# ViskaWei/VIT

Measured on AMD Instinct MI355X. Metric: images/sec ViT-B/16 224^2 bf16 train step, higher is better.
Workload: dtype bf16

## Files before the change

### vit_amd/csrc/gemm2.hip

```cpp
#include <algorithm>
#include <stdio.h>

#include "common.h"

namespace vit {

#define GLB_AS __attribute__((address_space(1)))

struct Gemm2Args {
  const char* A; const char* B; char* C;
  long lda, ldb, ldc;
  int M, N, K;
  int tiles_m, tiles_n, nblk;
  int splits, k_per_split;
  float* slab;
  const float* bias;
  const short* aux_in; short* aux_out; long ldaux;
  const float* residual; long ldres;
  float alpha;
  int act, c_dtype;
  DropCfg drop;
  int rpb, orb, roff;
  int drs;
  int lin_split;
  float* colsum_part;
  int grp2;
  const float* rope_cos; const float* rope_sin;
  int rope_T, rope_dh, rope_cols;
};

__device__ __forceinline__ int tr_swz2(int k) { return ((k & 3) | (((k >> 3) & 1) << 2)) << 2; }

template <int WM, int WN, int CW, int EPI>
__device__ __forceinline__ void tile_epilogue(f32x4 (&acc)[WM][WN], char* scr, const Gemm2Args& p, int m0, int n0,
                                              int split, int lane) {
  const int l15 = lane & 15, lg = lane >> 4;
  constexpr int CPR = CW / 4;
  constexpr int RPI = 64 / CPR;
  float* slab = p.splits > 1 ? p.slab + (long)split * p.M * p.N : nullptr;
#pragma unroll
  for (int i = 0; i < WM; ++i) {
#pragma unroll
    for (int jc = 0; jc < (WN * 16) / CW; ++jc) {
#pragma unroll
      for (int jj = 0; jj < CW / 16; ++jj) {
        const int c16 = jj * 4 + lg;
        *(f32x4*)(scr + l15 * (CW * 4) + ((c16 ^ (l15 & (CPR - 1))) << 4)) = acc[i][jc * (CW / 16) + jj];
        acc[i][jc * (CW / 16) + jj] = (f32x4){0.f, 0.f, 0.f, 0.f};
      }
#pragma unroll
      for (int rr = 0; rr < 16 / RPI; ++rr) {
        const int row = rr * RPI + lane / CPR, c16 = lane % CPR;
        f32x4 v = *(const f32x4*)(scr + row * (CW * 4) + ((c16 ^ (row & (CPR - 1))) << 4));
        const int m = m0 + i * 16 + row, n = n0 + jc * CW + c16 * 4;
        if (slab) {
          *(f32x4*)(slab + (long)m * p.N + n) = v;
          continue;
        }
        long orow = m;
        if (p.rpb > 0) {
          const int b = m / p.rpb;
          orow = (long)b * p.orb + (m - b * p.rpb) + p.roff;
        }
        v *= p.alpha;
        if (p.bias) v += *(const f32x4*)(p.bias + n);
        if (EPI == 1) {
          f32x4 sv = v;
          if (p.act == VIT_ACT_GELU_GRAD) {
#pragma unroll
            for (int r = 0; r < 4; ++r) {
              float g_, d_;
              gelu_both(v[r], g_, d_);
              v[r] = g_;
              sv[r] = d_;
            }
          } else {
#pragma unroll
            for (int r = 0; r < 4; ++r) v[r] = gelu_erf(v[r]);
          }
          if (p.aux_out) {
            u32x2 pk = {pack2bf(sv[0], sv[1]), pack2bf(sv[2], sv[3])};
            *(u32x2*)(p.aux_out + orow * p.ldaux + n) = pk;
          }
        } else if (EPI == 2) {
          bf16x4 u = *(const bf16x4*)(p.aux_in + orow * p.ldaux + n);
          if (p.act == VIT_ACT_MUL_AUX) {
#pragma unroll
            for (int r = 0; r < 4; ++r) v[r] *= bf2f(u[r]);
          } else {
#pragma unroll
            for (int r = 0; r < 4; ++r) v[r] *= dgelu_erf(bf2f(u[r]));
          }
        }
        if (p.drop.thr) {
          float k0, k1, k2, k3;
          const unsigned long long krow = (unsigned long long)orow * (unsigned)p.drs;
          drop_pair(p.drop, krow, (unsigned)n, k0, k1);
          drop_pair(p.drop, krow, (unsigned)n + 2, k2, k3);
          v[0] *= k0; v[1] *= k1; v[2] *= k2; v[3] *= k3;
        }
        if (p.residual) v += *(const f32x4*)(p.residual + orow * p.ldres + n);
        if (p.c_dtype == VIT_BF16) {
          u32x2 pk = {pack2bf(v[0], v[1]), pack2bf(v[2], v[3])};
          *(u32x2*)(p.C + (orow * p.ldc + n) * 2) = pk;
        } else {
          *(f32x4*)(p.C + (orow * p.ldc + n) * 4) = v;
        }
      }
    }
  }
}

int launch_splitk_reduce(const float* slab, float* C, long ldc, int M, int N, int splits, float alpha, int accumulate,
                         hipStream_t st);

template <int FAST, int NI>
__device__ __forceinline__ void pp_epilogue(f32x4 (&acc)[NI][4], char* scr, const Gemm2Args& p, int m0, int n0, int split,
                                            int lane) {
  const int l15 = lane & 15, lg = lane >> 4;
  if (FAST == 7) {
    float* cf = p.splits > 1 ? p.slab + (long)split * p.M * p.N : (float*)p.C;
    const long ldc = p.splits > 1 ? (long)p.N : p.ldc;
    const int n = n0 + l15 * 4;
#pragma unroll
    for (int i = 0; i < NI; ++i) {
#pragma unroll
      for (int j = 0; j < 4; ++j) {
        *(f32x4*)(scr + l15 * 256 + (((j * 4 + lg) ^ l15) << 4)) = acc[i][j];
        acc[i][j] = (f32x4){0.f, 0.f, 0.f, 0.f};
      }
#pragma unroll
      for (int rr = 0; rr < 4; ++rr) {
        const int row = rr * 4 + lg;
        *(f32x4*)(cf + (long)(m0 + i * 16 + row) * ldc + n) = *(const f32x4*)(scr + row * 256 + ((l15 ^ row) << 4));
      }
    }
    return;
  }
  const int cg = lane & 7, rsub = lane >> 3;
  const int n = n0 + cg * 8;
  const __amdgpu_buffer_rsrc_t rc_ = make_rsrc(p.C, (unsigned long long)p.M * p.ldc * 2);
  const __amdgpu_buffer_rsrc_t ra_ = make_rsrc(p.aux_out ? (const void*)p.aux_out : (const void*)p.C, (unsigned long long)p.M * p.ldaux * 2);
#define EPI_STORE_C(M_, PK) __builtin_amdgcn_raw_buffer_store_b128(PK, rc_, (unsigned)(((M_) * p.ldc + n) * 2), 0, 16)
#define EPI_STORE_AUX(M_, PK) __builtin_amdgcn_raw_buffer_store_b128(PK, ra_, (unsigned)(((M_) * p.ldaux + n) * 2), 0, 16)
  f32x4 bv0 = (f32x4){0.f, 0.f, 0.f, 0.f}, bv1 = bv0;
  if ((FAST == 3 || FAST == 4 || FAST == 8) && p.bias) {
    bv0 = *(const f32x4*)(p.bias + n);
    bv1 = *(const f32x4*)(p.bias + n + 4);
  }
  float cs[8] = {0.f, 0.f, 0.f, 0.f, 0.f, 0.f, 0.f, 0.f};
  const bool want_cs = p.colsum_part != nullptr;
  u32x4 au[4][2];
  f32x4 rc0, rc1, rs0, rs1, k8c0, k8c1, k8s0, k8s1;
  int rt = 0;
  const int rope_peer = (lane ^ (p.rope_dh >> 4)) << 2;
  if (FAST == 8 && n0 < p.rope_cols) {
    const int hl_ = p.rope_dh >> 4, hd = p.rope_dh >> 1, io = (cg & (hl_ - 1)) * 8;
    rt = (m0 + rsub) % p.rope_T;
    const long to = (long)rt * hd + io, t8 = 8L * hd + io;
    rc0 = *(const f32x4*)(p.rope_cos + to); rc1 = *(const f32x4*)(p.rope_cos + to + 4);
    rs0 = *(const f32x4*)(p.rope_sin + to); rs1 = *(const f32x4*)(p.rope_sin + to + 4);
    k8c0 = *(const f32x4*)(p.rope_cos + t8); k8c1 = *(const f32x4*)(p.rope_cos + t8 + 4);
    k8s0 = *(const f32x4*)(p.rope_sin + t8); k8s1 = *(const f32x4*)(p.rope_sin + t8 + 4);
  }
  const __amdgpu_buffer_rsrc_t rx_ = make_rsrc(p.aux_in ? (const void*)p.aux_in : (const void*)p.C, (unsigned long long)p.M * p.ldaux * 2);
#pragma unroll
  for (int i = 0; i < NI; ++i) {
    if (FAST == 5 && (i & 3) == 0) {
#pragma unroll
      for (int ii = 0; ii < 4; ++ii)
#pragma unroll
        for (int rr = 0; rr < 2; ++rr)
          au[ii][rr] = __builtin_amdgcn_raw_buffer_load_b128(rx_, (unsigned)(((long)(m0 + (i + ii) * 16 + rr * 8 + rsub) * p.ldaux + n) * 2), 0, 18);
    }
    f32x4 v[2][2];
#pragma unroll
    for (int j = 0; j < 4; ++j) {
      *(f32x4*)(scr + l15 * 256 + (((j * 4 + lg) ^ l15) << 4)) = acc[i][j];
      acc[i][j] = (f32x4){0.f, 0.f, 0.f, 0.f};
    }
#pragma unroll
    for (int rr = 0; rr < 2; ++rr) {
      const int row = rr * 8 + rsub;
      v[rr][0] = *(const f32x4*)(scr + row * 256 + (((2 * cg) ^ row) << 4));
      v[rr][1] = *(const f32x4*)(scr + row * 256 + (((2 * cg + 1) ^ row) << 4));
    }
#pragma unroll
    for (int rr = 0; rr < 2; ++rr) {
      const long m = m0 + i * 16 + rr * 8 + rsub;
      float o[8];
#pragma unroll
      for (int r = 0; r < 4; ++r) {
        o[r] = v[rr][0][r] + bv0[r];
        o[4 + r] = v[rr][1][r] + bv1[r];
      }
      if (FAST == 4) {
        float sv[8];
        if (p.act == VIT_ACT_GELU_GRAD) {
#pragma unroll
          for (int r = 0; r < 8; r += 2) {
            f32x2 g_, d_;
            gelu_both2((f32x2){o[r], o[r + 1]}, g_, d_);
            o[r] = g_[0]; o[r + 1] = g_[1];
            sv[r] = d_[0]; sv[r + 1] = d_[1];
          }
        } else {
#pragma unroll
          for (int r = 0; r < 8; r += 2) {
            sv[r] = o[r]; sv[r + 1] = o[r + 1];
            const f32x2 g_ = gelu_erf2((f32x2){o[r], o[r + 1]});
            o[r] = g_[0]; o[r + 1] = g_[1];
          }
        }
        if (p.aux_out) {
          u32x4 pk = {pack2bf(sv[0], sv[1]), pack2bf(sv[2], sv[3]), pack2bf(sv[4], sv[5]), pack2bf(sv[6], sv[7])};
          EPI_STORE_AUX(m, pk);
        }
      }
      if (FAST == 5) {
        const u32x4 u = au[i & 3][rr];
        if (p.act == VIT_ACT_MUL_AUX) {
#pragma unroll
          for (int r = 0; r < 4; ++r) {
            o[2 * r] *= __builtin_bit_cast(float, u[r] << 16);
            o[2 * r + 1] *= __builtin_bit_cast(float, u[r] & 0xFFFF0000u);
          }
        } else {
#pragma unroll
          for (int r = 0; r < 4; ++r) {
            o[2 * r] *= dgelu_erf(__builtin_bit_cast(float, u[r] << 16));
            o[2 * r + 1] *= dgelu_erf(__builtin_bit_cast(float, u[r] & 0xFFFF0000u));
          }
        }
      }
      if (FAST == 8 && n0 < p.rope_cols) {
        const int hl = p.rope_dh >> 4;
        const float sg = (cg & hl) ? 1.f : -1.f;
        const f32x4 c0 = rc0, c1 = rc1, s0 = rs0, s1 = rs1;
        float px[8];
#pragma unroll
        for (int r = 0; r < 8; ++r)
          px[r] = __builtin_bit_cast(float, __builtin_amdgcn_ds_bpermute(rope_peer, __builtin_bit_cast(int, o[r])));
#pragma unroll
        for (int r = 0; r < 4; ++r) {
          o[r] = fmaf(o[r], c0[r], sg * px[r] * s0[r]);
          o[4 + r] = fmaf(o[4 + r], c1[r], sg * px[4 + r] * s1[r]);
        }
        rt += 8;
        const bool wrapped = rt >= p.rope_T;
        if (wrapped) rt -= p.rope_T;
        {
          const f32x4 nc0 = rc0 * k8c0 - rs0 * k8s0, ns0 = rs0 * k8c0 + rc0 * k8s0;
          const f32x4 nc1 = rc1 * k8c1 - rs1 * k8s1, ns1 = rs1 * k8c1 + rc1 * k8s1;
          rc0 = nc0; rs0 = ns0; rc1 = nc1; rs1 = ns1;
        }
        if (__builtin_amdgcn_ballot_w64(wrapped)) {
          const long to = (long)rt * (p.rope_dh >> 1) + (cg & (hl - 1)) * 8;
          rc0 = *(const f32x4*)(p.rope_cos + to); rc1 = *(const f32x4*)(p.rope_cos + to + 4);
          rs0 = *(const f32x4*)(p.rope_sin + to); rs1 = *(const f32x4*)(p.rope_sin + to + 4);
        }
      }
      if (FAST == 3 && p.drop.thr) {
#pragma unroll
        for (int r = 0; r < 4; ++r) {
          float k0, k1;
          drop_pair(p.drop, (unsigned long long)m, (unsigned)n + 2 * r, k0, k1);
          o[2 * r] *= k0;
          o[2 * r + 1] *= k1;
        }
      }
      u32x4 pk = {pack2bf(o[0], o[1]), pack2bf(o[2], o[3]), pack2bf(o[4], o[5]), pack2bf(o[6], o[7])};
      EPI_STORE_C(m, pk);
      if (want_cs) {
#pragma unroll
        for (int r = 0; r < 4; ++r) {
          cs[2 * r] += __builtin_bit_cast(float, pk[r] << 16);
          cs[2 * r + 1] += __builtin_bit_cast(float, pk[r] & 0xFFFF0000u);
        }
      }
    }
  }
  if (p.colsum_part) {
#pragma unroll
    for (int r = 0; r < 8; ++r) {
      float v = cs[r];
      v += __shfl_xor(v, 8, 64);
      v += __shfl_xor(v, 16, 64);
      v += __shfl_xor(v, 32, 64);
      cs[r] = v;
    }
    if (lane < 8) {
      float* dst = p.colsum_part + (long)(m0 >> 7) * p.N + n;
      *(f32x4*)dst = (f32x4){cs[0], cs[1], cs[2], cs[3]};
      *(f32x4*)(dst + 4) = (f32x4){cs[4], cs[5], cs[6], cs[7]};
    }
  }
#undef EPI_STORE_C
#undef EPI_STORE_AUX
}

template <int A_T, int B_T, int EPI, int NSLOT>
__global__ __launch_bounds__(512, 2) void gemm3_kernel(Gemm2Args p) {
  resolve_drop(p.drop);
  constexpr int BM = 256, BN = 256, BK = 64;
  constexpr int HALF = 128 * BK * 2;
  static_assert(NSLOT == 8, "the ring arithmetic below is for 8 slots (two K-tiles of four half-tiles)");
  constexpr int DEPTH = NSLOT - 3, INFL = 2 * (DEPTH - 1);
  constexpr int SCR = 4096, CW = 64;
  constexpr int XA0 = 0, XB0 = 1, XB1 = 2, XA1 = 3;
  constexpr int RELAX = INFL + (((EPI >= 3 && EPI <= 6) || EPI == 8) ? 16 : 32);
  extern __shared__ __attribute__((aligned(16))) char smem[];

  const int tid = threadIdx.x, lane = tid & 63;
  const int wave = __builtin_amdgcn_readfirstlane(tid >> 6);
  const int wr = wave >> 2, wc = wave & 3, grp = wr;
  const int l15 = lane & 15, lg = lane >> 4;

  const int ntile = p.tiles_m * p.tiles_n;
  int split = blockIdx.y, bx = blockIdx.x;
  if (p.lin_split) {
    const int total = ntile * p.splits, lin = blockIdx.x;
    const int q = total >> 3, r = total & 7, xcd = lin & 7, within = lin >> 3;
    const int pos = (xcd < r ? xcd * (q + 1) : r * (q + 1) + (xcd - r) * q) + within;
    split = pos / ntile;
    bx = pos - split * ntile;
  }
  const int k_begin = split * p.k_per_split;
  const int k_end = min(p.K, k_begin + p.k_per_split);
  const int nk = (k_end - k_begin) / BK;
  const int nblk = p.nblk;
  const int my_tiles = (ntile - bx + nblk - 1) / nblk;
  const int T = my_tiles * nk;

  int offA[2], offB[2];
#pragma unroll
  for (int i = 0; i < 2; ++i) {
    if (A_T == 0) {
      const int rimg = i * 64 + wave * 8 + (lane >> 3);
      offA[i] = (i * 128 + wave * 8 + (lane >> 3)) * (int)p.lda + (((lane & 7) ^ ((rimg >> 1) & 7)) << 3);
    } else {
      const int k = i * 32 + wave * 4 + (lane >> 4);
      const int c16 = (lane & 15) ^ (tr_swz2(k) >> 1);
      offA[i] = k * (int)p.lda + (c16 >> 3) * 128 + ((c16 & 7) << 3);
    }
    if (B_T == 0) {
      const int rimg = i * 64 + wave * 8 + (lane >> 3);
      offB[i] = ((rimg >> 5) * 64 + (rimg & 31)) * (int)p.ldb + (((lane & 7) ^ ((rimg >> 1) & 7)) << 3);
    } else {
      const int k = i * 32 + wave * 4 + (lane >> 4);
      const int c16 = (lane & 15) ^ (tr_swz2(k) >> 1);
      offB[i] = k * (int)p.ldb + (c16 >> 2) * 64 + ((c16 & 3) << 3);
    }
  }
  const long halfA = (A_T == 0) ? 64 * p.lda : 64, halfB = (B_T == 0) ? 32 * p.ldb : 32;

  auto tile_coords = [&](int j, int& tm, int& tn) {
    const int round0 = j * nblk;
    const int n_here = min(nblk, ntile - round0);
    const int q = n_here >> 3, r = n_here & 7, xcd = bx & 7, within = bx >> 3;
    const int pos = (xcd < r ? xcd * (q + 1) : r * (q + 1) + (xcd - r) * q) + within;
    if (p.grp2) {
      const int hgrp = n_here >> 1, hn = p.tiles_n >> 1;
      const int g = pos >= hgrp;
      const int u = (round0 >> 1) + (g ? pos - hgrp : pos);
      tm = u / hn;
      tn = g * hn + (u - tm * hn);
      return;
    }
    const int t = p.lin_split ? bx : round0 + pos;
    tm = t / p.tiles_n;
    tn = t - tm * p.tiles_n;
  };
  const long dA = (A_T == 0) ? (long)BK * 2 : (long)BK * p.lda * 2;
  const long dB = (B_T == 0) ? (long)BK * 2 : (long)BK * p.ldb * 2;
  int cj = 0, ckt = 0;
  const char *ca, *cb;
  auto tile_bases = [&](int j) {
    int tm, tn;
    tile_coords(j, tm, tn);
    ca = (A_T == 0) ? p.A + ((long)tm * BM * p.lda + k_begin) * 2 : p.A + ((long)k_begin * p.lda + (long)tm * BM) * 2;
    cb = (B_T == 0) ? p.B + ((long)tn * BN * p.ldb + k_begin) * 2 : p.B + ((long)k_begin * p.ldb + (long)tn * BN) * 2;
  };
  tile_bases(0);
  auto cursor_next = [&](const char*& ab, const char*& bb) {
    ab = ca;
    bb = cb;
    if (++ckt == nk) {
      if (cj + 1 < my_tiles) {
        ++cj;
        ckt = 0;
        tile_bases(cj);
      } else {
        ckt = nk - 1;
      }
    } else {
      ca += dA;
      cb += dB;
    }
  };
  unsigned dofs = 0;
  const unsigned smem_a = lds_addr_of(smem) + wave * 1024;
  auto issue_half = [&](const char* base, long half_off, const int (&off)[2]) {
    const unsigned dst = smem_a + dofs;
    dofs = (dofs + HALF) & (NSLOT * HALF - 1);
    const char* sb = base + half_off * 2;
    lds_dma16_s(sb, (unsigned)off[0] * 2u, dst);
    lds_dma16_s(sb, (unsigned)off[1] * 2u, dst + 8192);
  };

  const int tq = l15 >> 2, tp = l15 & 3;
  const int tr_f = (tq | ((lg & 1) << 2)) << 2;
  int kc_off[2];
#pragma unroll
  for (int s = 0; s < 2; ++s) kc_off[s] = l15 * 128 + (((s * 4 + lg) ^ (l15 >> 1)) << 4);
  auto read_frag = [&](const char* img, int trans, int base16, int s) -> bf16x8 {
    if (!trans) {
      return *(const bf16x8*)(img + base16 * (BK * 2) + kc_off[s]);
    } else {
      const char* pa = img + (s * 32 + lg * 8 + tq) * 256 + ((((base16 >> 2) + tp) ^ tr_f) << 3);
      bf16x4 lo = __builtin_amdgcn_ds_read_tr16_b64_v4i16((LDS_AS bf16x4*)pa);
      bf16x4 hi = __builtin_amdgcn_ds_read_tr16_b64_v4i16((LDS_AS bf16x4*)(pa + 4 * 256));
      return (bf16x8){lo[0], lo[1], lo[2], lo[3], hi[0], hi[1], hi[2], hi[3]};
    }
  };

  f32x4 acc[8][4];
#pragma unroll
  for (int i = 0; i < 8; ++i)
#pragma unroll
    for (int j = 0; j < 4; ++j) acc[i][j] = (f32x4){0.f, 0.f, 0.f, 0.f};
  bf16x8 af[4][2], b0[2][2], b1[2][2];

#define PP_READ_A(IMG)                                                                           \
  _Pragma("unroll") for (int i_ = 0; i_ < 4; ++i_) _Pragma("unroll") for (int s_ = 0; s_ < 2; ++s_) \
      af[i_][s_] = read_frag(IMG, A_T, wr * 64 + i_ * 16, s_);
#define PP_READ_B(BF, IMG)                                                                       \
  _Pragma("unroll") for (int j_ = 0; j_ < 2; ++j_) _Pragma("unroll") for (int s_ = 0; s_ < 2; ++s_) \
      BF[j_][s_] = read_frag(IMG, B_T, wc * 32 + j_ * 16, s_);
#define PP_MFMA(HA, HB, BF)                                                                      \
  __builtin_amdgcn_sched_barrier(0);                                                             \
  __builtin_amdgcn_s_barrier();                                                                  \
  asm volatile("s_waitcnt lgkmcnt(0)" ::: "memory");                                             \
  __builtin_amdgcn_sched_barrier(0);                                                             \
  __builtin_amdgcn_s_setprio(1);                                                                 \
  _Pragma("unroll") for (int s_ = 0; s_ < 2; ++s_) _Pragma("unroll") for (int i_ = 0; i_ < 4; ++i_) \
      _Pragma("unroll") for (int j_ = 0; j_ < 2; ++j_)                                            \
          acc[HA * 4 + i_][HB * 2 + j_] =                                                        \
              __builtin_amdgcn_mfma_f32_16x16x32_bf16(BF[j_][s_], af[i_][s_], acc[HA * 4 + i_][HB * 2 + j_], 0, 0, 0); \
  __builtin_amdgcn_s_setprio(0);                                                                 \
  __builtin_amdgcn_sched_barrier(0);                                                             \
  __builtin_amdgcn_s_barrier();
#define PP_STAGE(BASE, HOFF, OFF)                                                                \
  {                                                                                              \
  issue_half(BASE, HOFF, OFF);                                                                   \
  asm volatile("s_cmp_lg_u32 %0, 0\n\t"                                                          \
               "s_cbranch_scc1 .Lpp_relaxed_%=\n\t"                                              \
               "s_waitcnt vmcnt(%1)\n\t"                                                         \
               "s_branch .Lpp_waited_%=\n"                                                       \
               ".Lpp_relaxed_%=:\n\t"                                                            \
               "s_waitcnt vmcnt(%2)\n"                                                           \
               ".Lpp_waited_%=:" ::"s"(relaxed), "n"(INFL), "n"(RELAX) : "scc", "memory");        \
  }
#define PP_KTILE4                                                                                \
  PP_READ_B(b0, sp + XB0 * HALF)                                                                 \
  PP_READ_A(sp + XA0 * HALF)                                                                     \
  PP_STAGE(bb1, halfB, offB)                                                                     \
  PP_MFMA(0, 0, b0)                                                                              \
  PP_READ_B(b1, sp + XB1 * HALF)                                                                 \
  PP_STAGE(a1, halfA, offA)                                                                      \
  PP_MFMA(0, 1, b1)                                                                              \
  PP_READ_A(sp + XA1 * HALF)                                                                     \
  PP_STAGE(a2, 0, offA)                                                                          \
  PP_MFMA(1, 1, b1)                                                                              \
  PP_STAGE(bb2, 0, offB)                                                                         \
  PP_MFMA(1, 0, b0)
#define PP_LOADED(RX)                                                                            \
  asm volatile("s_cmp_lg_u32 %0, 0\n\t"                                                          \
               "s_cbranch_scc1 .Lpp_relaxed_%=\n\t"                                              \
               "s_waitcnt vmcnt(%1)\n\t"                                                         \
               "s_branch .Lpp_waited_%=\n"                                                       \
               ".Lpp_relaxed_%=:\n\t"                                                            \
               "s_waitcnt vmcnt(%2)\n"                                                           \
               ".Lpp_waited_%=:\n\t"                                                             \
               "s_waitcnt lgkmcnt(0)" ::"s"(relaxed), "n"(INFL), "n"(RX) : "scc", "memory");
#define PP_MFMA2(HA, BFA, HBA, BFB, HBB)                                                         \
  __builtin_amdgcn_sched_barrier(0);                                                             \
  __builtin_amdgcn_s_barrier();                                                                  \
  __builtin_amdgcn_sched_barrier(0);                                                             \
  __builtin_amdgcn_s_setprio(1);                                                                 \
  _Pragma("unroll") for (int s_ = 0; s_ < 2; ++s_) _Pragma("unroll") for (int i_ = 0; i_ < 4; ++i_) \
      _Pragma("unroll") for (int j_ = 0; j_ < 2; ++j_)                                            \
          acc[HA * 4 + i_][HBA * 2 + j_] =                                                       \
              __builtin_amdgcn_mfma_f32_16x16x32_bf16(BFA[j_][s_], af[i_][s_], acc[HA * 4 + i_][HBA * 2 + j_], 0, 0, 0); \
  _Pragma("unroll") for (int s_ = 0; s_ < 2; ++s_) _Pragma("unroll") for (int i_ = 0; i_ < 4; ++i_) \
      _Pragma("unroll") for (int j_ = 0; j_ < 2; ++j_)                                            \
          acc[HA * 4 + i_][HBB * 2 + j_] =                                                       \
              __builtin_amdgcn_mfma_f32_16x16x32_bf16(BFB[j_][s_], af[i_][s_], acc[HA * 4 + i_][HBB * 2 + j_], 0, 0, 0); \
  __builtin_amdgcn_s_setprio(0);                                                                 \
  __builtin_amdgcn_sched_barrier(0);                                                             \
  __builtin_amdgcn_s_barrier();
#define PP_KTILE2                                                                                \
  PP_READ_B(b0, sp + XB0 * HALF)                                                                 \
  PP_READ_A(sp + XA0 * HALF)                                                                     \
  PP_READ_B(b1, sp + XB1 * HALF)                                                                 \
  issue_half(a1, halfA, offA);                                                                   \
  PP_LOADED(RELAX)                                                                               \
  PP_MFMA2(0, b0, 0, b1, 1)                                                                      \
  PP_READ_A(sp + XA1 * HALF)                                                                     \
  issue_half(a2, 0, offA);                                                                       \
  issue_half(bb2, 0, offB);                                                                      \
  issue_half(bb2, halfB, offB);                                                                  \
  PP_LOADED(RELAX)                                                                               \
  PP_MFMA2(1, b1, 1, b0, 0)
  constexpr bool MERGED = A_T || B_T;

  static_assert(DEPTH == 5, "stage schedule written out for the 8-slot ring");
  const char *a1, *bb1, *a2, *bb2;
  {
    const char *a0, *bb0;
    cursor_next(a0, bb0);
    issue_half(a0, 0, offA);
    issue_half(bb0, 0, offB);
    issue_half(bb0, halfB, offB);
    issue_half(a0, halfA, offA);
    cursor_next(a1, bb1);
    issue_half(a1, 0, offA);
    issue_half(bb1, 0, offB);
    if constexpr (MERGED) issue_half(bb1, halfB, offB);
    asm volatile("s_waitcnt vmcnt(%0)" ::"n"(INFL) : "memory");
    cursor_next(a2, bb2);
  }
  __builtin_amdgcn_s_barrier();
  if (grp == 1) __builtin_amdgcn_s_barrier();

  unsigned kb = 0;
  int relaxed = 0;
  for (int jt = 0; jt < my_tiles; ++jt) {
    for (int kt = 0; kt < nk; ++kt) {
      const char* sp = smem + kb;
      if constexpr (MERGED) {
        PP_KTILE2
      } else {
        PP_KTILE4
      }
      relaxed = 0;
      a1 = a2;
      bb1 = bb2;
      cursor_next(a2, bb2);
      kb ^= 4 * HALF;
    }
    {
      int tm, tn;
      tile_coords(jt, tm, tn);
      if (grp == 0) __builtin_amdgcn_s_barrier();
      char* scr = smem + 8 * HALF + wave * SCR;
      if constexpr (EPI >= 3) pp_epilogue<EPI, 8>(acc, scr, p, tm * BM + wr * 128, tn * BN + wc * 64, split, lane);
      else tile_epilogue<8, 4, CW, EPI>(acc, scr, p, tm * BM + wr * 128, tn * BN + wc * 64, split, lane);
      if (grp == 1) __builtin_amdgcn_s_barrier();
      relaxed = 1;
    }
  }
  if (grp == 0) __builtin_amdgcn_s_barrier();
#undef PP_READ_A
#undef PP_READ_B
#undef PP_MFMA
#undef PP_STAGE
#undef PP_KTILE2
#undef PP_KTILE4
#undef PP_LOADED
#undef PP_MFMA2
  asm volatile("s_waitcnt vmcnt(0)" ::: "memory");
}

template <int AT, int BT, int EPI>
static int launch_stag(const Gemm2Args& a, dim3 grid, hipStream_t st) {
  constexpr int smem = 160 * 1024;
  static bool attr_done = false;
  auto fn = gemm3_kernel<AT, BT, EPI, 8>;
  if (!attr_done) {
    VIT_HIP(hipFuncSetAttribute((const void*)fn, hipFuncAttributeMaxDynamicSharedMemorySize, smem));
    attr_done = true;
  }
  hipLaunchKernelGGL(fn, grid, dim3(512), smem, st, a);
  VIT_LAUNCH_CHECK();
  return VIT_OK;
}
static int launch_stag_cfg(const Gemm2Args& a, int at, int bt, int epi, dim3 grid, hipStream_t st) {
  if (epi == 1) return launch_stag<0, 0, 1>(a, grid, st);
  if (epi == 2) return launch_stag<0, 1, 2>(a, grid, st);
  if (epi == 3) return launch_stag<0, 0, 3>(a, grid, st);
  if (epi == 4) return launch_stag<0, 0, 4>(a, grid, st);
  if (epi == 5) return launch_stag<0, 1, 5>(a, grid, st);
  if (epi == 6) return launch_stag<0, 1, 6>(a, grid, st);
  if (epi == 8) return launch_stag<0, 0, 8>(a, grid, st);
  if (epi == 7) return launch_stag<1, 1, 7>(a, grid, st);
  if (!at && !bt) return launch_stag<0, 0, 0>(a, grid, st);
  if (!at && bt) return launch_stag<0, 1, 0>(a, grid, st);
  if (at && !bt) return launch_stag<1, 0, 0>(a, grid, st);
  return launch_stag<1, 1, 0>(a, grid, st);
}

int g_gemm2_mode = 1;

static void pp_split_plan(int slots, int ntile, int K, int split_k, int* splits_out, int* kps_out) {
  const int ktiles = K / 64;
  int splits = split_k;
  if (splits < 0) {
    splits = 1;
    if (ntile < slots) splits = std::min(std::max(1, slots / ntile), std::max(1, ktiles / 8));
  }
  if (splits < 1) splits = 1;
  if (splits > ktiles) splits = ktiles;
  const int kps = cdiv(ktiles, splits) * 64;
  *splits_out = cdiv(K, kps);
  *kps_out = kps;
}

static bool pp_shape_ok(long M, long N, long K, long lda, long ldb) {
  if (g_gemm2_mode == 0) return false;
  if (M % 256 || N % 256 || K % 64) return false;
  if (lda * 256 >= (1L << 30) || ldb * 256 >= (1L << 30)) return false;
  return true;
}

bool pp_plan(vit_handle h, const vit_gemm_desc* d, GemmPlan* pl) {
  if (!pp_shape_ok(d->M, d->N, d->K, d->lda, d->ldb)) return false;
  int epi = 0;
  if (d->act == VIT_ACT_GELU || d->act == VIT_ACT_GELU_GRAD) {
    if (d->a_trans || d->b_trans) return false;
    epi = 1;
  } else if (d->act == VIT_ACT_DGELU || d->act == VIT_ACT_MUL_AUX) {
    if (d->a_trans || !d->b_trans) return false;
    epi = 2;
  }
  const int slots = ctx_num_cus(h);
  const int tiles_m = d->M / 256, tiles_n = d->N / 256, ntile = tiles_m * tiles_n;
  int splits, kps;
  pp_split_plan(slots, ntile, d->K, d->split_k, &splits, &kps);
  if (splits > 1 && !(d->c_dtype == VIT_F32 && !d->bias && d->act == VIT_ACT_NONE && d->dropout_p == 0.f && !d->residual &&
                      d->rows_per_batch == 0)) return false;
  if (d->accumulate && splits == 1 && !(d->c_dtype == VIT_F32 && !d->residual && d->rows_per_batch == 0)) return false;

  int nblk = std::min(ntile, slots);
  dim3 grid(nblk, splits);
  int lin_split = 0;
  if (splits > 1 && nblk == ntile) {
    lin_split = 1;
    grid = dim3(ntile * splits, 1);
  }
  int epi5 = epi;
  const bool residual = d->residual || (d->accumulate && splits == 1);
  const unsigned drop_thr = pl->drop.thr;
  const bool plain = !residual && d->rows_per_batch == 0 && pl->drs == 1 && d->alpha == 1.0f;
  if (epi == 1 && plain && d->bias && d->c_dtype == VIT_BF16 && !drop_thr && splits == 1) epi5 = 4;
  else if (epi == 2 && plain && !d->bias && d->c_dtype == VIT_BF16 && !drop_thr && splits == 1) epi5 = 5;
  else if (epi == 0 && plain && d->c_dtype == VIT_BF16 && !d->a_trans && !d->b_trans && splits == 1) epi5 = 3;
  else if (epi == 0 && plain && !d->bias && !drop_thr && d->c_dtype == VIT_BF16 && !d->a_trans && d->b_trans &&
           splits == 1) epi5 = 6;
  else if (epi == 0 && plain && !d->bias && !drop_thr && d->c_dtype == VIT_F32 && d->a_trans && d->b_trans) epi5 = 7;
  if (d->rope_cos) {
    if (epi5 == 3 && !drop_thr && (d->rope_dh == 16 || d->rope_dh == 32 || d->rope_dh == 64) && (d->rope_cols % 64) == 0 &&
        d->rope_T >= 9)
      epi5 = 8;
  }
  if (((epi5 >= 3 && epi5 <= 6) || epi5 == 8) &&
      ((unsigned long long)d->M * d->ldc * 2 >= 0x7FFFFFF0ull ||
       ((d->aux_out || d->aux_in) && (unsigned long long)d->M * d->ldaux * 2 >= 0x7FFFFFF0ull)))
    epi5 = epi;
  if (splits == 1 && ntile > slots) {
    nblk = cdiv(ntile, cdiv(ntile, slots));
    grid = dim3(nblk, splits);
  }
  int grp2 = 0;
  if (splits == 1 && (tiles_n % 2) == 0 && (size_t)d->N * d->K * 2 > (size_t)4 << 20 && ntile > slots && (ntile % 2) == 0) {
    grp2 = 1;
    if (nblk & 1) {
      nblk += 1;
      grid = dim3(nblk, splits);
    }
  }
  pl->core = GEMM_PP;
  pl->a_t = d->a_trans; pl->b_t = d->b_trans; pl->epi = epi5;
  pl->splits = splits; pl->k_per_split = kps;
  pl->tiles_m = tiles_m; pl->tiles_n = tiles_n;
  pl->grid = grid; pl->nblk = nblk; pl->lin_split = lin_split; pl->grp2 = grp2;
  if (d->colsum_out) {
    pl->colsum = (epi5 == 3 || epi5 == 5 || epi5 == 6) ? PASS_FUSED : PASS_BEHIND;
    if (pl->colsum == PASS_FUSED) pl->colsum_bytes = (size_t)tiles_m * 2 * d->N * sizeof(float);
  }
  if (d->rope_cos) pl->rope = epi5 == 8 ? PASS_FUSED : PASS_BEHIND;
  snprintf(pl->symbol, sizeof(pl->symbol), "gemm3_kernel<%d, %d, %d, %d>", pl->a_t, pl->b_t, epi5, 8);
  return true;
}

int pp_launch(const GemmPlan& pl, const vit_gemm_desc* d, hipStream_t st) {
  Gemm2Args a;
  fill_gemm_args(a, pl, d);
  a.nblk = pl.nblk; a.lin_split = pl.lin_split; a.grp2 = pl.grp2;
  a.colsum_part = pl.colsum == PASS_FUSED ? (float*)pl.ws : nullptr;
  a.rope_cos = d->rope_cos; a.rope_sin = d->rope_sin; a.rope_T = d->rope_T; a.rope_dh = d->rope_dh; a.rope_cols = d->rope_cols;
  int r = launch_stag_cfg(a, pl.a_t, pl.b_t, pl.epi, pl.grid, st);
  if (r == VIT_OK && a.colsum_part)
    r = launch_reduce_partials(a.colsum_part, a.tiles_m * 2, d->N, d->colsum_out, d->N, d->colsum_out, pl.grad_accumulate, st);
  if (r == VIT_OK && pl.splits > 1)
    r = launch_splitk_reduce(a.slab, (float*)d->C, (long)d->ldc, d->M, d->N, pl.splits, d->alpha, pl.accumulate, st);
  return r;
}


__global__ __launch_bounds__(256) void dw_rows_kernel(const short* __restrict__ dy, long ldy, const short* __restrict__ x,
                                                      long ldx, float* __restrict__ dW, long ldw, int B, int s, int kps,
                                                      int splits, int accumulate) {
  constexpr int R = 128;
  __shared__ __attribute__((aligned(16))) short ys[R][64];
  __shared__ __attribute__((aligned(16))) short xs[R][64];
  const int t = threadIdx.x, lane = t & 63, wave = t >> 6, l15 = lane & 15, lg = lane >> 4;
  const int wn = (wave >> 1) * 32, wk = (wave & 1) * 32;
  const int n0 = blockIdx.x * 64, k0 = blockIdx.y * 64;
  f32x4 acc[2][2], tot[2][2];
#pragma unroll
  for (int i = 0; i < 2; ++i)
#pragma unroll
    for (int j = 0; j < 2; ++j) acc[i][j] = tot[i][j] = (f32x4){0.f, 0.f, 0.f, 0.f};
  int sp = 0;
  int bend = (int)min((long)B, ((long)(sp + 1) * kps + s - 1) / s);
  auto flush = [&]() {
#pragma unroll
    for (int i = 0; i < 2; ++i)
#pragma unroll
      for (int j = 0; j < 2; ++j) {
        tot[i][j] = sp == 0 ? acc[i][j] : tot[i][j] + acc[i][j];
        acc[i][j] = (f32x4){0.f, 0.f, 0.f, 0.f};
      }
    ++sp;
    bend = sp >= splits - 1 ? B : (int)min((long)B, ((long)(sp + 1) * kps + s - 1) / s);
  };
  if (splits == 1) bend = B;
  const int lr = t >> 3, lc = (t & 7) * 8;
  for (int b0 = 0; b0 < B; b0 += R) {
    __syncthreads();
    {
      u32x4 vy[R / 32], vx[R / 32];
#pragma unroll
      for (int q = 0; q < R / 32; ++q) {
        const int b = b0 + lr + 32 * q;
        vy[q] = vx[q] = (u32x4){0u, 0u, 0u, 0u};
        if (b < B) {
          vy[q] = *(const u32x4*)(dy + (long)b * ldy + n0 + lc);
          vx[q] = *(const u32x4*)(x + (long)b * ldx + k0 + lc);
        }
      }
#pragma unroll
      for (int q = 0; q < R / 32; ++q) {
        *(u32x4*)&ys[lr + 32 * q][lc] = vy[q];
        *(u32x4*)&xs[lr + 32 * q][lc] = vx[q];
      }
    }
    __syncthreads();
    const int nb = min(R, B - b0);
    int bb = 0;
    while (bb < nb) {
      while (b0 + bb >= bend) flush();
      const int seg = min(nb, bend - b0);
#pragma unroll 4
      for (; bb < seg; ++bb) {
        bf16x8 yf[2], xf[2];
#pragma unroll
        for (int i = 0; i < 2; ++i) {
          yf[i] = (bf16x8){0, 0, 0, 0, 0, 0, 0, 0};
          xf[i] = (bf16x8){0, 0, 0, 0, 0, 0, 0, 0};
          if (lg == 0) {
            yf[i][0] = ys[bb][wn + i * 16 + l15];
            xf[i][0] = xs[bb][wk + i * 16 + l15];
          }
        }
#pragma unroll
        for (int i = 0; i < 2; ++i)
#pragma unroll
          for (int j = 0; j < 2; ++j) acc[i][j] = __builtin_amdgcn_mfma_f32_16x16x32_bf16(yf[i], xf[j], acc[i][j], 0, 0, 0);
      }
    }
  }
  while (sp < splits) flush();
#pragma unroll
  for (int i = 0; i < 2; ++i)
#pragma unroll
    for (int j = 0; j < 2; ++j)
#pragma unroll
      for (int r = 0; r < 4; ++r) {
        float* o = dW + (long)(n0 + wn + i * 16 + 4 * lg + r) * ldw + k0 + wk + j * 16 + l15;
        *o = accumulate ? *o + tot[i][j][r] : tot[i][j][r];
      }
}

__global__ void colsum_rows_part_kernel(const short* __restrict__ a, long lda, float* __restrict__ part, int nblk, int N,
                                        int B, int s) {
  const long i = blockIdx.x * (long)blockDim.x + threadIdx.x;
  if (i >= (long)nblk * N) return;
  const int p = (int)(i / N), n = (int)(i - (long)p * N);
  const int b0 = (int)(((long)p * 128 + s - 1) / s), b1 = (int)min((long)B, ((long)(p + 1) * 128 + s - 1) / s);
  float v = 0.f;
  for (int b = b0; b < b1; ++b) v += bf2f(a[(long)b * lda + n]);
  part[i] = v;
}

int colsum_strided(vit_handle h, const void* a, int a_dtype, int64_t lda, float* out, int rows, int cols, int64_t row_stride,
                   int held, int accumulate, hipStream_t st);

}

extern "C" {

int vit_linear_bwd_dw_rows(vit_handle h, const void* dy, int64_t ldy, const void* x, int64_t ldx, int dtype, float* dW,
                           int rows, int N, int K, int64_t row_stride, int64_t full_rows, vit_stream stream) {
  using namespace vit;
  VIT_CHECK(dy && x && dW, VIT_ERR_ARG, "vit_linear_bwd_dw_rows: null pointer");
  VIT_CHECK(rows > 0 && N > 0 && K > 0 && row_stride >= 1 && full_rows >= (int64_t)(rows - 1) * row_stride + 1 &&
                full_rows <= 0x7FFFFFFF && ldy >= N && ldx >= K,
            VIT_ERR_ARG, "vit_linear_bwd_dw_rows: rows=%d N=%d K=%d row_stride=%lld full_rows=%lld", rows, N, K,
            (long long)row_stride, (long long)full_rows);
  hipStream_t st = (hipStream_t)stream;
  vit_gemm_desc d = {};
  d.M = N; d.N = K; d.K = (int)full_rows; d.ab_dtype = dtype; d.a_trans = 1; d.b_trans = 1;
  d.A = dy; d.lda = ldy; d.B = x; d.ldb = ldx; d.C = dW; d.ldc = K; d.c_dtype = VIT_F32; d.alpha = 1.f; d.split_k = -1;
  if (dtype == VIT_BF16) {
    GemmPlan pl;
    const int rc = gemm_plan(h, &d, KRows{0, 0}, &pl);
    if (rc != VIT_OK) return rc;
    if (pl.core == GEMM_PP) {
      hipLaunchKernelGGL(dw_rows_kernel, dim3(N / 64, K / 64), dim3(256), 0, st, (const short*)dy, (long)ldy, (const short*)x,
                         (long)ldx, dW, (long)K, rows, (int)row_stride, pl.k_per_split, pl.splits, ctx_grad_accumulate(h));
      VIT_LAUNCH_CHECK();
      return VIT_OK;
    }
  }
  if (dtype == VIT_F32 && row_stride > 1 &&
      (unsigned long long)rows * (unsigned long long)std::max(ldy, ldx) * 4 < 0x7FFFFFF0ull)
    return gemm_launch(h, &d, st, (int)row_stride, rows);
  d.K = rows; d.split_k = 1;
  return gemm_launch(h, &d, st);
}

int vit_colsum_rows(vit_handle h, const void* a, int a_dtype, int64_t lda, float* out, int rows, int cols, int64_t row_stride,
                    int64_t full_rows, vit_stream stream) {
  using namespace vit;
  VIT_CHECK(a && out, VIT_ERR_ARG, "vit_colsum_rows: null pointer");
  VIT_CHECK(rows > 0 && cols > 0 && lda >= cols && row_stride >= 1 && full_rows >= (int64_t)(rows - 1) * row_stride + 1 &&
                full_rows <= 0x7FFFFFFF,
            VIT_ERR_ARG, "vit_colsum_rows: rows=%d cols=%d row_stride=%lld full_rows=%lld", rows, cols, (long long)row_stride,
            (long long)full_rows);
  hipStream_t st = (hipStream_t)stream;
  if (a_dtype == VIT_BF16 && pp_shape_ok(full_rows, cols, 64, 64, 64)) {
    const int nblk = (int)(full_rows / 128);
    float* part = (float*)ctx_claim(h, (size_t)nblk * cols * sizeof(float), "vit_colsum_rows");
    if (!part) return VIT_ERR_WORKSPACE;
    hipLaunchKernelGGL(colsum_rows_part_kernel, dim3((unsigned)cdiv((long)nblk * cols, 256)), dim3(256), 0, st,
                       (const short*)a, (long)lda, part, nblk, cols, rows, (int)row_stride);
    VIT_LAUNCH_CHECK();
    return launch_reduce_partials(part, nblk, cols, out, cols, out, ctx_grad_accumulate(h), st);
  }
  if (a_dtype == VIT_F32 && row_stride > 1)
    return colsum_strided(h, a, a_dtype, lda, out, (int)full_rows, cols, row_stride, rows, ctx_grad_accumulate(h), st);
  return vit_colsum(h, a, a_dtype, lda, out, rows, cols, ctx_grad_accumulate(h), stream);
}

}
```

Before: 7865.

## Template dw_rows kernel on tile shape, transpose staging for vector LDS reads

The strided-row weight-gradient kernel is templated on per-wave tile counts, and the host picks a tile shape (2x2, 1x3, 1x1) that balances block count against CU count. Shared-memory staging now transposes rows into column-major padded buffers, so each lane fetches 8 rows with one vector LDS read and prefetches the next chunk. The split-boundary check becomes an incrementing position counter. This is meant to cut scalar LDS loads and improve occupancy balance for small N×K, at the cost of packing/shuffle ALU work and more template instances.

Result: no change. 7894, median of 6 (+0.4%).

```diff
diff --git a/vit_amd/csrc/gemm2.hip b/vit_amd/csrc/gemm2.hip
--- a/vit_amd/csrc/gemm2.hip
+++ b/vit_amd/csrc/gemm2.hip
@@ -1,5 +1,6 @@
 #include <algorithm>
 #include <stdio.h>
+#include <type_traits>
 
 #include "common.h"
 
@@ -708,89 +709,144 @@
 }
 
 
+template <int TI, int TJ>
 __global__ __launch_bounds__(256) void dw_rows_kernel(const short* __restrict__ dy, long ldy, const short* __restrict__ x,
                                                       long ldx, float* __restrict__ dW, long ldw, int B, int s, int kps,
                                                       int splits, int accumulate) {
-  constexpr int R = 128;
-  __shared__ __attribute__((aligned(16))) short ys[R][64];
-  __shared__ __attribute__((aligned(16))) short xs[R][64];
+  constexpr int R = 128, RS = R * 2 + 16;
+  constexpr int NY = 32 * TI, NX = 32 * TJ;
+  __shared__ __attribute__((aligned(16))) char ys[(NY + 1) * RS];
+  __shared__ __attribute__((aligned(16))) char xs[(NX + 1) * RS];
   const int t = threadIdx.x, lane = t & 63, wave = t >> 6, l15 = lane & 15, lg = lane >> 4;
-  const int wn = (wave >> 1) * 32, wk = (wave & 1) * 32;
-  const int n0 = blockIdx.x * 64, k0 = blockIdx.y * 64;
-  f32x4 acc[2][2], tot[2][2];
-#pragma unroll
-  for (int i = 0; i < 2; ++i)
-#pragma unroll
-    for (int j = 0; j < 2; ++j) acc[i][j] = tot[i][j] = (f32x4){0.f, 0.f, 0.f, 0.f};
+  const int wn = (wave >> 1) * 16 * TI, wk = (wave & 1) * 16 * TJ;
+  const int n0 = blockIdx.x * NY, k0 = blockIdx.y * NX;
+  for (int i = t; i < RS / 4; i += 256) {
+    ((unsigned*)(ys + NY * RS))[i] = 0u;
+    ((unsigned*)(xs + NX * RS))[i] = 0u;
+  }
+  f32x4 acc[TI][TJ], tot[TI][TJ];
+#pragma unroll
+  for (int i = 0; i < TI; ++i)
+#pragma unroll
+    for (int j = 0; j < TJ; ++j) acc[i][j] = tot[i][j] = (f32x4){0.f, 0.f, 0.f, 0.f};
   int sp = 0;
-  int bend = (int)min((long)B, ((long)(sp + 1) * kps + s - 1) / s);
+  unsigned lim = splits > 1 ? (unsigned)kps : 0xFFFFFFFFu, pos = 0;
   auto flush = [&]() {
 #pragma unroll
-    for (int i = 0; i < 2; ++i)
-#pragma unroll
-      for (int j = 0; j < 2; ++j) {
+    for (int i = 0; i < TI; ++i)
+#pragma unroll
+      for (int j = 0; j < TJ; ++j) {
         tot[i][j] = sp == 0 ? acc[i][j] : tot[i][j] + acc[i][j];
         acc[i][j] = (f32x4){0.f, 0.f, 0.f, 0.f};
       }
     ++sp;
-    bend = sp >= splits - 1 ? B : (int)min((long)B, ((long)(sp + 1) * kps + s - 1) / s);
+    lim = sp >= splits - 1 ? 0xFFFFFFFFu : lim + kps;
   };
-  if (splits == 1) bend = B;
-  const int lr = t >> 3, lc = (t & 7) * 8;
+  const int sp_ = t & (R / 2 - 1), sc = t / (R / 2);
+  auto stage = [&](auto nc_, const short* __restrict__ src, long ld, int c0, char* dst, int b0) {
+    constexpr int NC = decltype(nc_)::value;
+    u32x4 e[NC], o[NC];
+    const int b = b0 + 2 * sp_;
+#pragma unroll
+    for (int q = 0; q < NC; ++q) {
+      e[q] = o[q] = (u32x4){0u, 0u, 0u, 0u};
+      const short* g = src + (long)b * ld + c0 + (sc + 4 * q) * 8;
+      if (b < B) e[q] = *(const u32x4*)g;
+      if (b + 1 < B) o[q] = *(const u32x4*)(g + ld);
+    }
+#pragma unroll
+    for (int q = 0; q < NC; ++q) {
+      char* d = dst + (sc + 4 * q) * 8 * RS + sp_ * 4;
+#pragma unroll
+      for (int j = 0; j < 4; ++j) {
+        *(unsigned*)(d + (2 * j) * RS) = (e[q][j] & 0xFFFFu) | (o[q][j] << 16);
+        *(unsigned*)(d + (2 * j + 1) * RS) = (e[q][j] >> 16) | (o[q][j] & 0xFFFF0000u);
+      }
+    }
+  };
+  int ya[TI], xa[TJ];
+#pragma unroll
+  for (int i = 0; i < TI; ++i) ya[i] = (lg == 0 ? wn + i * 16 + l15 : NY) * RS;
+#pragma unroll
+  for (int j = 0; j < TJ; ++j) xa[j] = (lg == 0 ? wk + j * 16 + l15 : NX) * RS;
+  unsigned zy[TI][3], zx[TJ][3];
+#pragma unroll
+  for (int q = 0; q < 3; ++q) {
+#pragma unroll
+    for (int i = 0; i < TI; ++i) asm volatile("v_mov_b32 %0, 0" : "=v"(zy[i][q]));
+#pragma unroll
+    for (int j = 0; j < TJ; ++j) asm volatile("v_mov_b32 %0, 0" : "=v"(zx[j][q]));
+  }
   for (int b0 = 0; b0 < B; b0 += R) {
     __syncthreads();
-    {
-      u32x4 vy[R / 32], vx[R / 32];
-#pragma unroll
-      for (int q = 0; q < R / 32; ++q) {
-        const int b = b0 + lr + 32 * q;
-        vy[q] = vx[q] = (u32x4){0u, 0u, 0u, 0u};
-        if (b < B) {
-          vy[q] = *(const u32x4*)(dy + (long)b * ldy + n0 + lc);
-          vx[q] = *(const u32x4*)(x + (long)b * ldx + k0 + lc);
-        }
-      }
-#pragma unroll
-      for (int q = 0; q < R / 32; ++q) {
-        *(u32x4*)&ys[lr + 32 * q][lc] = vy[q];
-        *(u32x4*)&xs[lr + 32 * q][lc] = vx[q];
-      }
-    }
+    stage(std::integral_constant<int, TI>{}, dy, ldy, n0, ys, b0);
+    stage(std::integral_constant<int, TJ>{}, x, ldx, k0, xs, b0);
     __syncthreads();
     const int nb = min(R, B - b0);
-    int bb = 0;
-    while (bb < nb) {
-      while (b0 + bb >= bend) flush();
-      const int seg = min(nb, bend - b0);
-#pragma unroll 4
-      for (; bb < seg; ++bb) {
-        bf16x8 yf[2], xf[2];
-#pragma unroll
-        for (int i = 0; i < 2; ++i) {
-          yf[i] = (bf16x8){0, 0, 0, 0, 0, 0, 0, 0};
-          xf[i] = (bf16x8){0, 0, 0, 0, 0, 0, 0, 0};
-          if (lg == 0) {
-            yf[i][0] = ys[bb][wn + i * 16 + l15];
-            xf[i][0] = xs[bb][wk + i * 16 + l15];
-          }
-        }
-#pragma unroll
-        for (int i = 0; i < 2; ++i)
-#pragma unroll
-          for (int j = 0; j < 2; ++j) acc[i][j] = __builtin_amdgcn_mfma_f32_16x16x32_bf16(yf[i], xf[j], acc[i][j], 0, 0, 0);
+    u32x4 yn[TI], xn[TJ];
+#pragma unroll
+    for (int i = 0; i < TI; ++i) yn[i] = *(const u32x4*)(ys + ya[i]);
+#pragma unroll
+    for (int j = 0; j < TJ; ++j) xn[j] = *(const u32x4*)(xs + xa[j]);
+    for (int c = 0; c * 8 < nb; ++c) {
+      u32x4 yv[TI], xv[TJ];
+#pragma unroll
+      for (int i = 0; i < TI; ++i) {
+        yv[i] = yn[i];
+        yn[i] = *(const u32x4*)(ys + ya[i] + (c + 1) * 16);
+      }
+#pragma unroll
+      for (int j = 0; j < TJ; ++j) {
+        xv[j] = xn[j];
+        xn[j] = *(const u32x4*)(xs + xa[j] + (c + 1) * 16);
+      }
+#pragma unroll
+      for (int r = 0; r < 8; ++r) {
+        while (pos >= lim) flush();
+        pos += s;
+        bf16x8 yf[TI], xf[TJ];
+#pragma unroll
+        for (int i = 0; i < TI; ++i) {
+          const unsigned w = yv[i][r >> 1];
+          yf[i] = __builtin_bit_cast(bf16x8, (u32x4){(r & 1) ? w >> 16 : w & 0xFFFFu, zy[i][0], zy[i][1], zy[i][2]});
+        }
+#pragma unroll
+        for (int j = 0; j < TJ; ++j) {
+          const unsigned w = xv[j][r >> 1];
+          xf[j] = __builtin_bit_cast(bf16x8, (u32x4){(r & 1) ? w >> 16 : w & 0xFFFFu, zx[j][0], zx[j][1], zx[j][2]});
+        }
+#pragma unroll
+        for (int i = 0; i < TI; ++i)
+#pragma unroll
+          for (int j = 0; j < TJ; ++j) acc[i][j] = __builtin_amdgcn_mfma_f32_16x16x32_bf16(yf[i], xf[j], acc[i][j], 0, 0, 0);
       }
     }
   }
   while (sp < splits) flush();
 #pragma unroll
-  for (int i = 0; i < 2; ++i)
-#pragma unroll
-    for (int j = 0; j < 2; ++j)
+  for (int i = 0; i < TI; ++i)
+#pragma unroll
+    for (int j = 0; j < TJ; ++j)
 #pragma unroll
       for (int r = 0; r < 4; ++r) {
         float* o = dW + (long)(n0 + wn + i * 16 + 4 * lg + r) * ldw + k0 + wk + j * 16 + l15;
         *o = accumulate ? *o + tot[i][j][r] : tot[i][j][r];
       }
+}
+
+static void dw_rows_shape(int cus, int N, int K, int* ti, int* tj) {
+  static const int forms[3][2] = {{2, 2}, {1, 3}, {1, 1}};
+  long best = -1;
+  for (const auto& f : forms) {
+    if (N % (32 * f[0]) || K % (32 * f[1])) continue;
+    const long blocks = (long)(N / (32 * f[0])) * (K / (32 * f[1]));
+    const long cost = cdiv(blocks, (long)cus) * f[0] * f[1];
+    if (best < 0 || cost < best) {
+      best = cost;
+      *ti = f[0];
+      *tj = f[1];
+    }
+  }
 }
 
 __global__ void colsum_rows_part_kernel(const short* __restrict__ a, long lda, float* __restrict__ part, int nblk, int N,
@@ -828,7 +884,10 @@
     const int rc = gemm_plan(h, &d, KRows{0, 0}, &pl);
     if (rc != VIT_OK) return rc;
     if (pl.core == GEMM_PP) {
-      hipLaunchKernelGGL(dw_rows_kernel, dim3(N / 64, K / 64), dim3(256), 0, st, (const short*)dy, (long)ldy, (const short*)x,
+      int ti = 1, tj = 1;
+      dw_rows_shape(ctx_num_cus(h), N, K, &ti, &tj);
+      auto fn = ti == 2 ? dw_rows_kernel<2, 2> : tj == 3 ? dw_rows_kernel<1, 3> : dw_rows_kernel<1, 1>;
+      hipLaunchKernelGGL(fn, dim3(N / (32 * ti), K / (32 * tj)), dim3(256), 0, st, (const short*)dy, (long)ldy, (const short*)x,
                          (long)ldx, dW, (long)K, rows, (int)row_stride, pl.k_per_split, pl.splits, ctx_grad_accumulate(h));
       VIT_LAUNCH_CHECK();
       return VIT_OK;
```
